# GANtastic3/MaskCycleGAN-VC

Measured on AMD Instinct MI355X. Metric: train iters/s (full G+D step), 80x64 mel bs=1, higher is better.
Workload: dtype f32

## Files before the change

### maskcyclegan-vc_amd/csrc/net.hip

```cpp
#include "mcvc_common.h"
#include "twin.h"
#include "pack.h"
#include "misc.h"
#include "trunk.h"
#include "wino.h"
#include "wino4.h"
#include "sgemm.h"
#include "sampler.h"
#include "audio.h"
#include "vocoder.h"
#include "../../include/mcvc.h"
#include <string.h>
#include <algorithm>
#include <map>
#include <mutex>
#include <vector>

static int g_deterministic = [] { const char* e = getenv("MCVC_DETERMINISTIC"); return (e && atoi(e) != 0) ? 1 : 0; }();
int mcvc_deterministic() { return g_deterministic; }

namespace {

constexpr float kInEps = 1e-5f;

// ... 1020 lines not shown
            PackJob q{}; q.kind = PACK_TRUNK_T; q.param = c.wi[br]; q.dst = c.off_tk; q.Cout = c.Cout; q.Cin = c.Cin; q.KW = c.KW;
            q.ld = c.cout_tot * c.KW; q.co_off = br * c.Cout;
            add_job(t, q, cdiv_i(c.Cin, 32), cdiv_i(c.Cout, 32));
        }
        if (c.igemm && (sets & 4) == 0) {
            PackJob fi{}; fi.kind = PACK_FWD_TAP; fi.param = c.wi[br]; fi.dst = c.off_ifwd; fi.Cout = c.Cout; fi.K = K; fi.ld = c.cout_pk;
            fi.co_off = br * c.Cout; fi.KW = c.KH * c.KW;
            if (fw) add_job(t, fi, cdiv_i(K, 32), cdiv_i(c.Cout, 32));
            t.bytes += 4.0 * fw * 2.0 * c.Cout * K; t.wbytes += 4.0 * fw * c.Cout * K;
        }
        if (c.wino3) {
            PackJob w3{}; w3.kind = PACK_WINO3_D; w3.param = c.wi[br]; w3.dst = c.off_w3; w3.Cout = c.Cout; w3.Cin = c.Cin; w3.ld = c.mg_ld;
            w3.xi_stride = c.w3_xi; w3.co_off = br * c.Cout;
            if (bw) add_job(t, w3, cdiv_i(c.Cin, 256), c.Cout);
            PackJob w3f{}; w3f.kind = PACK_WINO3_F; w3f.param = c.wi[br]; w3f.dst = c.off_w3f; w3f.Cout = c.Cout; w3f.Cin = c.Cin; w3f.ld = c.cout_pk;
            w3f.xi_stride = c.w3f_xi; w3f.co_off = br * c.Cout;
            if (fw) add_job(t, w3f, cdiv_i(c.Cout, 256), c.Cin);
            t.bytes += 4.0 * (fw + bw) * (25.0 + 64.0) * c.Cout * c.Cin; t.wbytes += 4.0 * (fw + bw) * 64.0 * c.Cout * c.Cin;
        }
        if (c.wino3 && w43) {
            PackJob w3{}; w3.kind = PACK_WINO43_D; w3.param = c.wi[br]; w3.dst = c.off_w43; w3.Cout = c.Cout; w3.Cin = c.Cin; w3.ld = c.mg_ld;
            w3.xi_stride = c.w3_xi; w3.co_off = br * c.Cout;
            if (bw) add_job(t, w3, cdiv_i(c.Cin, 256), c.Cout);
            PackJob w3f{}; w3f.kind = PACK_WINO43_F; w3f.param = c.wi[br]; w3f.dst = c.off_w43f; w3f.Cout = c.Cout; w3f.Cin = c.Cin; w3f.ld = c.cout_pk;
            w3f.xi_stride = c.w3f_xi; w3f.co_off = br * c.Cout;
            if (fw) add_job(t, w3f, cdiv_i(c.Cout, 256), c.Cin);
            t.bytes += 4.0 * (fw + bw) * (25.0 + 144.0) * c.Cout * c.Cin; t.wbytes += 4.0 * (fw + bw) * 144.0 * c.Cout * c.Cin;
        }
        if (c.wino && w4) {
            PackJob wf{}; wf.kind = PACK_WINO4_F; wf.param = c.wi[br]; wf.dst = c.off_w4f; wf.Cout = c.Cout; wf.Cin = c.Cin; wf.ld = c.cout_pk;
            wf.xi_stride = c.wf_xi; wf.co_off = br * c.Cout;
            if (fw) add_job(t, wf, cdiv_i(c.Cout, 256), c.Cin);
            PackJob wd{}; wd.kind = PACK_WINO4_D; wd.param = c.wi[br]; wd.dst = c.off_w4d; wd.Cout = c.Cout; wd.Cin = c.Cin; wd.ld = c.cin_pk;
            wd.xi_stride = c.wd_xi; wd.co_off = br * c.Cout;
            if (bw) add_job(t, wd, cdiv_i(c.Cin, 256), c.Cout);
            t.bytes += 4.0 * (fw + bw) * (25.0 + 64.0) * c.Cout * c.Cin; t.wbytes += 4.0 * (fw + bw) * 64.0 * c.Cout * c.Cin;
        }
        if (c.wino && w2) {
            PackJob wf{}; wf.kind = PACK_WINO_F; wf.param = c.wi[br]; wf.dst = c.off_wf; wf.Cout = c.Cout; wf.Cin = c.Cin; wf.ld = c.cout_pk;
            wf.xi_stride = c.wf_xi; wf.co_off = br * c.Cout;
            if (fw) add_job(t, wf, cdiv_i(c.Cout, 256), c.Cin);
            PackJob wd{}; wd.kind = PACK_WINO_D; wd.param = c.wi[br]; wd.dst = c.off_wd; wd.Cout = c.Cout; wd.Cin = c.Cin; wd.ld = c.cin_pk;
            wd.xi_stride = c.wd_xi; wd.co_off = br * c.Cout;
            if (bw) add_job(t, wd, cdiv_i(c.Cin, 256), c.Cout);
            t.bytes += 4.0 * (fw + bw) * (25.0 + 36.0) * c.Cout * c.Cin; t.wbytes += 4.0 * (fw + bw) * 36.0 * c.Cout * c.Cin;
        }
        t.bytes += skip_direct ? 8.0 * c.Cout : 4.0 * ((c.off_tk >= 0 ? 6.0 : 4.0) * c.Cout * K + 2.0 * c.Cout);
        t.wbytes += skip_direct ? 4.0 * c.Cout : 4.0 * ((c.off_tk >= 0 ? 3.0 : 2.0) * c.Cout * K + c.Cout);
    }
}

struct DevPackTable { PackJob* jobs; PackDgradArgs* dga; int njobs, nblocks; double bytes; std::vector<int> used; };

template <class Build>
static const DevPackTable* dev_pack_table(int kind, Build&& build, int* err)
{
    static std::mutex mu;
    static std::map<std::pair<int, int>, DevPackTable> cache;
    int dev = 0;
    if (hipGetDevice(&dev) != hipSuccess) { *err = MCVC_ERR_INVALID; return nullptr; }
    std::lock_guard<std::mutex> lk(mu);
    auto it = cache.find({dev, kind});
    if (it != cache.end()) return &it->second;
    PackTable t;
    build(t);
    DevPackTable d{};
    d.njobs = (int)t.jobs.size(); d.nblocks = t.nblocks; d.bytes = t.bytes;
    hipError_t e = hipMalloc((void**)&d.jobs, t.jobs.size() * sizeof(PackJob));
    if (e == hipSuccess) e = hipMalloc((void**)&d.dga, t.dga.size() * sizeof(PackDgradArgs));
    if (e == hipSuccess) e = hipMemcpy(d.jobs, t.jobs.data(), t.jobs.size() * sizeof(PackJob), hipMemcpyHostToDevice);
    if (e == hipSuccess) e = hipMemcpy(d.dga, t.dga.data(), t.dga.size() * sizeof(PackDgradArgs), hipMemcpyHostToDevice);
    if (e != hipSuccess) { *err = (int)e; return nullptr; }
    for (const PackJob& j : t.jobs) d.used.push_back(j.param);
    return &cache.emplace(std::make_pair(dev, kind), std::move(d)).first->second;
}

static int pack_net(const DevPackTable* t, const float* const* params, float* packed, hipStream_t s)
{
    PackPtrs ptrs{};
    for (int i : t->used) { if (i < 0 || i >= 128) return MCVC_ERR_INVALID; ptrs.p[i] = params[i]; }
    return mcvc_pack_net_launch(t->jobs, t->njobs, t->nblocks, t->dga, ptrs, packed, t->bytes, s);
}

struct DevUpdTable { UpdOwner* owners; PackJob* jobs; PackDgradArgs* dga; int nown, nblocks; double adam_floats, pack_bytes; std::vector<int> used;
                     std::vector<long long> sizes; };

template <class Build, class InRange>
static const DevUpdTable* dev_upd_table(int kind, Build&& build, const long long* numel, int nparams, InRange&& in_range, int* err)
{
    static std::mutex mu;
    static std::map<std::pair<int, int>, DevUpdTable> cache;
    int dev = 0;
    if (hipGetDevice(&dev) != hipSuccess) { *err = MCVC_ERR_INVALID; return nullptr; }
    std::lock_guard<std::mutex> lk(mu);
    auto it = cache.find({dev, kind});
    if (it != cache.end()) return &it->second;
    PackTable t;
    build(t);
    std::vector<PackJob> jobs;
    std::vector<UpdOwner> owners;
    DevUpdTable d{};
    int nblocks = 0;
    for (int prm = 0; prm < nparams && prm < 128; ++prm) {
        std::vector<PackJob> mine;
        for (const PackJob& j : t.jobs) if (j.param == prm) mine.push_back(j);
        if (!in_range(prm)) { if (!mine.empty()) { *err = MCVC_ERR_INVALID; return nullptr; } continue; }
        if (numel[prm] <= 0) { if (!mine.empty()) { *err = MCVC_ERR_INVALID; return nullptr; } continue; }
        UpdOwner o{};
        o.param = prm; o.block0 = nblocks; o.e0 = (int)jobs.size(); o.ne = (int)mine.size();
        bool weight = false;
        for (const PackJob& j : mine) weight = weight || j.kind != PACK_COPY;
        if (!weight) {
            o.flat = 1; o.Cout = (int)numel[prm]; o.Cin = o.taps = 1; o.gx = 1;
            for (const PackJob& j : mine) if (j.Cout != o.Cout) { *err = MCVC_ERR_INVALID; return nullptr; }
            nblocks += cdiv_i(o.Cout, 256);
        } else {
            const PackJob& j0 = mine[0];
            o.Cout = j0.Cout; o.Cin = j0.Cin; o.taps = j0.taps;
            for (const PackJob& j : mine) if (j.kind == PACK_COPY || j.Cout != o.Cout || j.Cin != o.Cin || j.taps != o.taps) { *err = MCVC_ERR_INVALID; return nullptr; }
            for (const PackJob& j : mine) if (j.kind >= PACK_WINO_F && j.kind <= PACK_WINO43_F && j.taps != 25) { *err = MCVC_ERR_INVALID; return nullptr; }
            if ((long long)o.Cout * o.Cin * o.taps != numel[prm]) { *err = MCVC_ERR_INVALID; return nullptr; }
            int cb = 32, ib = 32;
            static const int cb25 = mcvc_knob("MCVC_UPD_CB25", 32);
            if (o.taps == 25) { cb = cb25 == 16 ? 16 : 32; ib = 16; }
            else if (o.taps == 3) ib = 64;
            else if (o.taps == 1) ib = 128;
            else if (o.taps > 25) ib = 16;
            o.CB = cb < o.Cout ? cb : o.Cout; o.IB = ib < o.Cin ? ib : o.Cin;
            if ((size_t)o.CB * mcvc_upd_pitch(o.IB, o.taps) * sizeof(float) > kUpdLds) { *err = MCVC_ERR_INVALID; return nullptr; }
            o.vec4 = ((o.IB * o.taps) % 4 == 0 && (o.Cin % o.IB) == 0 && ((long long)o.Cin * o.taps) % 4 == 0) ? 1 : 0;
            o.gx = cdiv_i(o.Cin, o.IB);
            nblocks += o.gx * cdiv_i(o.Cout, o.CB);
        }
        d.adam_floats += (double)numel[prm];
        for (const PackJob& j : mine) jobs.push_back(j);
        owners.push_back(o);
        d.used.push_back(prm); d.sizes.push_back(numel[prm]);
    }
    if (jobs.size() != t.jobs.size() || owners.empty()) { *err = MCVC_ERR_INVALID; return nullptr; }
    d.nown = (int)owners.size(); d.nblocks = nblocks;
    d.pack_bytes = t.wbytes;
    if (jobs.empty()) jobs.push_back(PackJob{});
    if (t.dga.empty()) t.dga.push_back(PackDgradArgs{});
    hipError_t e = hipMalloc((void**)&d.owners, owners.size() * sizeof(UpdOwner));
    if (e == hipSuccess) e = hipMalloc((void**)&d.jobs, jobs.size() * sizeof(PackJob));
    if (e == hipSuccess) e = hipMalloc((void**)&d.dga, t.dga.size() * sizeof(PackDgradArgs));
    if (e == hipSuccess) e = hipMemcpy(d.owners, owners.data(), owners.size() * sizeof(UpdOwner), hipMemcpyHostToDevice);
    if (e == hipSuccess) e = hipMemcpy(d.jobs, jobs.data(), jobs.size() * sizeof(PackJob), hipMemcpyHostToDevice);
    if (e == hipSuccess) e = hipMemcpy(d.dga, t.dga.data(), t.dga.size() * sizeof(PackDgradArgs), hipMemcpyHostToDevice);
    if (e != hipSuccess) { *err = (int)e; return nullptr; }
    return &cache.emplace(std::make_pair(dev, kind), std::move(d)).first->second;
}

struct UpdOpt { const float* flat; const float* grad; const float* grad2; const float* exp_avg; const float* exp_avg_sq;
                float lr, beta1, beta2, eps; int step; float grad_scale; int zero_grads; };

static int update_net(const DevUpdTable* t, const float* const* params, const long long* numel, float* packed, const UpdOpt& o, hipStream_t s)
{
    for (size_t k = 0; k < t->used.size(); ++k) if (numel[t->used[k]] != t->sizes[k]) return MCVC_ERR_INVALID;
    if (!o.flat || !o.grad || !o.exp_avg || !o.exp_avg_sq || o.step < 1) return MCVC_ERR_INVALID;
    if ((((uintptr_t)o.flat | (uintptr_t)o.grad | (uintptr_t)o.grad2 | (uintptr_t)o.exp_avg | (uintptr_t)o.exp_avg_sq) & 15) != 0) return MCVC_ERR_INVALID;
    PackPtrs ptrs{};
    for (int i : t->used) { if (i < 0 || i >= 128 || !params[i] || (((uintptr_t)params[i]) & 15) != 0) return MCVC_ERR_INVALID; ptrs.p[i] = params[i]; }
    UpdAdam ad{};
    ad.d_g = o.grad - o.flat; ad.d_m = o.exp_avg - o.flat; ad.d_v = o.exp_avg_sq - o.flat;
    ad.has_g2 = o.grad2 ? 1 : 0; ad.d_g2 = o.grad2 ? o.grad2 - o.flat : 0;
    ad.zero = o.zero_grads;
    ad.c = mcvc_adam_coef(o.lr, o.beta1, o.beta2, o.eps, o.step, o.grad_scale);
    const double bytes = (28.0 + (o.grad2 ? 4.0 : 0.0) + (o.zero_grads ? (o.grad2 ? 8.0 : 4.0) : 0.0)) * t->adam_floats + t->pack_bytes;
    return mcvc_update_net_launch(t->owners, t->nown, t->nblocks, t->jobs, t->dga, ptrs, packed, ad, bytes, s);
}

static bool trunk_enabled()
{
    static const int en = mcvc_knob("MCVC_TRUNK", 1);
    return en != 0;
}

static int g_trunk_net = mcvc_knob("MCVC_TRUNK_NET", 1) != 0;
static bool trunk_net_enabled() { return g_trunk_net != 0; }
static bool trunk_bwd_net_enabled() { return g_trunk_net == 1; }

static bool trunk_fwd(Exec& ex, const ConvSpec& c, const float* const* P, int g0, int be0, int g1, int be1, const float* x, float* conv_out,
                      float* stats, float* y, long long y_sn, long long y_sc, const float* res, int B, int W4)
{
    const int mode = (c.nbr == 2) ? TRUNK_IN_GLU : TRUNK_IN;
    if (!trunk_enabled() || c.KH != 1 || !mcvc_trunk_applies(c.Cin, c.KW, c.Cout, B, W4, mode, 1)) return false;
    if (ex.dry) return true;
    TrunkArgs a{};
    a.a0 = P[c.wi[0]]; a.bias0 = P[c.bi[0]]; a.gamma0 = P[g0]; a.beta0 = P[be0];
    if (c.nbr == 2) { a.a1 = P[c.wi[1]]; a.bias1 = P[c.bi[1]]; a.gamma1 = P[g1]; a.beta1 = P[be1]; }
    a.x = x; a.x_sc = (long long)B * W4; a.x_sb = W4;
    a.Cin = c.Cin; a.KW = c.KW; a.K = c.Cin * c.KW; a.M = c.Cout; a.Mtot = c.cout_tot; a.B = B; a.T4 = W4; a.N = B * W4;
    a.conv_out = conv_out; a.c_sc = (long long)B * W4; a.c_sb = W4;
    a.stats = stats; a.y = y; a.res = res; a.y_sn = y_sn; a.y_sc = y_sc; a.eps = kInEps; a.mode = mode;
    ex.fail(mcvc_trunk_launch(a, 1, ex.s));
    return true;
}

static int trunk_pick_ksplit(int Cin, int KW, int M, int B, int W4, int must_split)
{
    int best = 0;
    for (int ks = 1; ks <= 64; ++ks) {
        if (!mcvc_trunk_applies(Cin, KW, M, B, W4, TRUNK_PLAIN, ks)) continue;
        if (best == 0) best = ks;
        if ((M / 16) * ks <= 512) best = ks;
    }
    (void)must_split;
    return best;
}

struct TrunkPre {
    int kind;
    const float* x; const float* stats;
    const float* g0; const float* b0; const float* g1; const float* b1;
    float* out;
    float* dg0; float* db0; float* dg1; float* db1;
    int xB;
};

static bool trunk_dgrad(Exec& ex, const ConvSpec& c, const float* packed, const float* dy, float* dx, int accumulate, int B, int W4,
                        int* nsplit = nullptr, const TrunkPre* pre = nullptr)
{
    if (!trunk_enabled() || c.off_tk < 0) return false;
    int ks = 1;
    if (!accumulate && mcvc_trunk_applies(c.cout_tot, c.KW, c.Cin, B, W4, TRUNK_PLAIN, 1)) ks = 1;
    else ks = trunk_pick_ksplit(c.cout_tot, c.KW, c.Cin, B, W4, 0);
    if (ks < 1) return false;
    if (!accumulate && ks > 1 && !nsplit) return false;
    const long long tot = (long long)c.Cin * B * W4;
    const bool slab_all = accumulate && ks > 1 && nsplit && mcvc_deterministic();
    if (ks > 1 && (!accumulate || nsplit)) {
        const long long need = (long long)(accumulate ? ks : ks - 1) * tot;
        if (need > ex.slab_need) ex.slab_need = need;
        if (!ex.dry && need > ex.slab_cap) { ex.fail(MCVC_ERR_WORKSPACE); return true; }
    }
    if (nsplit) *nsplit = slab_all ? ks + 1 : (accumulate ? 1 : ks);
    if (ex.dry) return true;
    TrunkArgs a{};
    a.a0 = packed + c.off_tk;
    a.x = dy; a.x_sc = (long long)B * W4; a.x_sb = W4;
    a.Cin = c.cout_tot; a.KW = c.KW; a.K = c.cout_tot * c.KW; a.M = c.Cin; a.Mtot = c.Cin; a.B = B; a.T4 = W4; a.N = B * W4;
    a.conv_out = dx; a.c_sc = (long long)B * W4; a.c_sb = W4; a.accumulate = accumulate; a.mode = TRUNK_PLAIN;
    a.slabs = ex.slabs; a.slab_stride = tot; a.slab_all = slab_all ? 1 : 0;
    if (pre) {
        a.pre = pre->kind; a.pre_C = (pre->kind == 2) ? c.cout_tot / 2 : c.cout_tot;
        a.pre_x = pre->x; a.pre_xB = pre->xB; a.pre_stats = pre->stats; a.pre_gamma0 = pre->g0; a.pre_beta0 = pre->b0; a.pre_gamma1 = pre->g1; a.pre_beta1 = pre->b1;
        a.pre_out = pre->out; a.pre_dgamma0 = pre->dg0; a.pre_dbeta0 = pre->db0; a.pre_dgamma1 = pre->dg1; a.pre_dbeta1 = pre->db1;
        wait_readers(ex, pre->out);
    }
    ex.fail(mcvc_trunk_launch(a, ks, ex.s));
    return true;
}
// ... 1612 lines not shown
```

### maskcyclegan-vc_amd/csrc/pack.h

```cpp
#pragma once
#include <hip/hip_runtime.h>

struct DgradClass {
    int nth, ntw;
    int khmax, kwmax;
    int pad_h, pad_w;
    int qh, qw;
    int su, sv;
    long long offset;
};

struct PackDgradArgs {
    int Cin, KH, KW;
    int step;
    int ld;
    int co_off;
    int merged;
    int mg_kh, mg_kw;
    int ncls;
    DgradClass cls[4];
    int tapmajor;
    int cout_rows;
};

int mcvc_pack_fwd_launch(const float* w, float* dst, int Cout, int K, int ld, int co_off, hipStream_t s);
int mcvc_pack_dgrad_launch(const float* w, float* dst, const PackDgradArgs& a, int Cout, hipStream_t s);
int mcvc_copy_launch(const float* src, float* dst, int n, hipStream_t s);

enum PackKind { PACK_FWD = 0, PACK_DGRAD = 1, PACK_COPY = 2, PACK_TRUNK_T = 3, PACK_WINO_F = 4, PACK_WINO_D = 5, PACK_WINO3_D = 6, PACK_WINO3_F = 7, PACK_WINO4_F = 8, PACK_WINO4_D = 9, PACK_WINO43_D = 10, PACK_WINO43_F = 11,
                PACK_FWD_TAP = 12 };
struct PackJob {
    int kind, param;
    int block0, gx;
    long long dst;
    int Cout, K, ld, co_off, KW, Cin;
    int dg;
    int taps;
    long long xi_stride;
};
struct PackPtrs { const float* p[128]; };
constexpr size_t kPackNetLds = 32 * 75 * sizeof(float);
int mcvc_pack_net_launch(const PackJob* d_jobs, int njobs, int nblocks, const PackDgradArgs* d_dga, const PackPtrs& ptrs, float* packed,
                         double bytes, hipStream_t s);
int mcvc_pack_trunk_t_launch(const float* w, float* dst, int Cout, int Cin, int KW, int ld, int co_off, hipStream_t s);

#include "misc.h"
struct UpdOwner {
    int param;
    int block0, gx;
    int Cout, Cin, taps;
    int CB, IB;
    int e0, ne;
    int flat;
    int vec4;
};
struct UpdAdam { long long d_g, d_g2, d_m, d_v; int has_g2, zero; AdamCoef c; };
static inline int mcvc_upd_pitch(int IB, int taps) { return ((IB * taps + 3) & ~3) + 1; }
constexpr size_t kUpdLds = 52 * 1024;
int mcvc_update_net_launch(const UpdOwner* d_owners, int nown, int nblocks, const PackJob* d_jobs, const PackDgradArgs* d_dga, const PackPtrs& ptrs,
                           float* packed, const UpdAdam& ad, double bytes, hipStream_t s);
```

### maskcyclegan-vc_amd/csrc/pack_kernels.hip

```cpp
#include "mcvc_common.h"
#include "pack.h"
#include "trace.h"
#include "launch.h"
#include "wino.h"
#include "wino4.h"

__device__ __forceinline__ void pack_fwd_tile(const float* __restrict__ w, float* __restrict__ dst, int Cout, int K, int ld, int co_off,
                                              int bx, int by, float* smem, int taps = 0)
{
    float (*tile)[33] = reinterpret_cast<float (*)[33]>(smem);
    const int k0 = bx * 32, c0 = by * 32;
    const int tx = threadIdx.x & 31, ty = threadIdx.x >> 5;
    for (int r = ty; r < 32; r += 8) {
        const int co = c0 + r, k = k0 + tx;
        tile[r][tx] = (co < Cout && k < K) ? w[(long long)co * K + k] : 0.f;
    }
    __syncthreads();
    for (int r = ty; r < 32; r += 8) {
        const int k = k0 + r, co = c0 + tx;
        if (k < K && co < Cout) {
            const int row = taps > 0 ? (k % taps) * (K / taps) + k / taps : k;
            dst[(long long)row * ld + co_off + co] = tile[tx][r];
        }
    }
}

__device__ __forceinline__ void pack_dgrad_tile(const float* __restrict__ w, float* __restrict__ dst, const PackDgradArgs& a, int bx, int by,
                                                float* lds)
{
    const int ci0 = bx * 32, co = by;
    const int khkw = a.KH * a.KW;
    int nci = a.Cin - ci0; if (nci > 32) nci = 32;
    const float* src = w + ((long long)co * a.Cin + ci0) * khkw;
    for (int i = threadIdx.x; i < nci * khkw; i += 256) lds[i] = src[i];
    __syncthreads();
    const int lane = threadIdx.x & 31, grp = threadIdx.x >> 5;
    for (int c = 0; c < a.ncls; ++c) {
        const int nt = a.cls[c].nth * a.cls[c].ntw;
        for (int t = grp; t < nt; t += 8) {
            const int u = t / a.cls[c].ntw, v = t - u * a.cls[c].ntw;
            const int kh = a.cls[c].khmax - a.step * u, kw = a.cls[c].kwmax - a.step * v;
            if (lane < nci) {
                const float wv = lds[lane * khkw + kh * a.KW + kw];
                if (a.tapmajor) {
                    dst[a.cls[c].offset + ((long long)t * a.cout_rows + a.co_off + co) * a.ld + ci0 + lane] = wv;
                } else if (a.merged) {
                    const long long row = ((long long)(a.co_off + co) * a.mg_kh + (u + a.cls[c].su)) * a.mg_kw + (v + a.cls[c].sv);
                    dst[row * a.ld + 4 * (ci0 + lane) + 2 * a.cls[c].qh + a.cls[c].qw] = wv;
                } else {
                    dst[a.cls[c].offset + ((long long)(a.co_off + co) * nt + t) * a.ld + ci0 + lane] = wv;
                }
            }
        }
    }
}

__device__ __forceinline__ void pack_trunk_t_tile(const float* __restrict__ w, float* __restrict__ dst, int Cout, int Cin, int KW, int ld,
                                                  int co_off, int bx, int by, float* smem)
{
    float (*tile)[33] = reinterpret_cast<float (*)[33]>(smem);
    const int ci0 = bx * 32, co0 = by * 32;
    const int tx = threadIdx.x & 31, ty = threadIdx.x >> 5;
    for (int kw = 0; kw < KW; ++kw) {
        for (int r = ty; r < 32; r += 8) {
            const int co = co0 + r, ci = ci0 + tx;
            tile[r][tx] = (co < Cout && ci < Cin) ? w[((long long)co * Cin + ci) * KW + kw] : 0.f;
        }
        __syncthreads();
        for (int r = ty; r < 32; r += 8) {
            const int ci = ci0 + r, co = co0 + tx;
            if (ci < Cin && co < Cout) dst[(long long)ci * ld + (long long)(co_off + co) * KW + (KW - 1 - kw)] = tile[tx][r];
        }
        __syncthreads();
    }
}

__global__ void __launch_bounds__(256) pack_fwd_kernel(const float* __restrict__ w, float* __restrict__ dst, int Cout, int K, int ld, int co_off)
{
    __shared__ float smem[32 * 33];
    pack_fwd_tile(w, dst, Cout, K, ld, co_off, blockIdx.x, blockIdx.y, smem);
}

__global__ void __launch_bounds__(256) pack_dgrad_kernel(const float* __restrict__ w, float* __restrict__ dst, PackDgradArgs a)
{
    extern __shared__ float lds[];
    pack_dgrad_tile(w, dst, a, blockIdx.x, blockIdx.y, lds);
}

__global__ void __launch_bounds__(256) pack_trunk_t_kernel(const float* __restrict__ w, float* __restrict__ dst, int Cout, int Cin, int KW, int ld,
                                                           int co_off)
{
    __shared__ float smem[32 * 33];
    pack_trunk_t_tile(w, dst, Cout, Cin, KW, ld, co_off, blockIdx.x, blockIdx.y, smem);
}

struct CopyKArgs { const float* src; float* dst; int n; };
__global__ void copy_kernel(const Twin<CopyKArgs> tw)
{
    const CopyKArgs ka_ = tw.v[blockIdx.z];
    const float* __restrict__ src = ka_.src;
    float* __restrict__ dst = ka_.dst;
    int n = ka_.n;
    const int i = blockIdx.x * blockDim.x + threadIdx.x;
    if (i < n) dst[i] = src[i];
}

struct PackNetKArgs { const PackJob* jobs; int njobs; const PackDgradArgs* dga; PackPtrs ptrs; float* packed; };
__global__ void __launch_bounds__(256) pack_net_kernel(const Twin<PackNetKArgs> tw)
{
    const PackNetKArgs& ka_ = tw.v[blockIdx.z];
    const PackJob* __restrict__ jobs = ka_.jobs;
    int njobs = ka_.njobs;
    const PackDgradArgs* __restrict__ dga = ka_.dga;
    const PackPtrs& ptrs = ka_.ptrs;
    float* __restrict__ packed = ka_.packed;
    extern __shared__ float lds[];
    const int blk = blockIdx.x;
    int lo = 0, hi = njobs - 1;
    while (lo < hi) { const int mid = (lo + hi + 1) >> 1; if (jobs[mid].block0 <= blk) lo = mid; else hi = mid - 1; }
    const PackJob j = jobs[lo];
    const int rel = blk - j.block0;
    const int bx = rel % j.gx, by = rel / j.gx;
    const float* w = ptrs.p[j.param];
    float* dst = packed + j.dst;
    switch (j.kind) {
    case PACK_FWD: pack_fwd_tile(w, dst, j.Cout, j.K, j.ld, j.co_off, bx, by, lds); break;
    case PACK_FWD_TAP: pack_fwd_tile(w, dst, j.Cout, j.K, j.ld, j.co_off, bx, by, lds, j.KW); break;
    case PACK_DGRAD: pack_dgrad_tile(w, dst, dga[j.dg], bx, by, lds); break;
    case PACK_TRUNK_T: pack_trunk_t_tile(w, dst, j.Cout, j.Cin, j.KW, j.ld, j.co_off, bx, by, lds); break;
    case PACK_WINO_F: wino_weight_tile(w, dst, j.Cout, j.Cin, j.ld, j.xi_stride, j.co_off, 0, bx, by); break;
    case PACK_WINO_D: wino_weight_tile(w, dst, j.Cout, j.Cin, j.ld, j.xi_stride, j.co_off, 1, bx, by); break;
    case PACK_WINO3_D: wino3_weight_tile(w, dst, j.Cout, j.Cin, j.ld, j.xi_stride, j.co_off, bx, by); break;
    case PACK_WINO3_F: wino3_weight_fwd_tile(w, dst, j.Cout, j.Cin, j.ld, j.xi_stride, j.co_off, bx, by); break;
    case PACK_WINO4_F: wino4_weight_tile(w, dst, j.Cout, j.Cin, j.ld, j.xi_stride, j.co_off, 0, bx, by); break;
    case PACK_WINO4_D: wino4_weight_tile(w, dst, j.Cout, j.Cin, j.ld, j.xi_stride, j.co_off, 1, bx, by); break;
    case PACK_WINO43_D: wino3_weight_tile_p<6>(w, dst, j.Cout, j.Cin, j.ld, j.xi_stride, j.co_off, bx, by); break;
    case PACK_WINO43_F: wino3_weight_fwd_tile_p<6>(w, dst, j.Cout, j.Cin, j.ld, j.xi_stride, j.co_off, bx, by); break;
    default: { const int i = rel * 256 + threadIdx.x; if (i < j.Cout) dst[i] = w[i]; } break;
    }
}

struct UpdTile { const float* lds; int pitch, taps, co0, ci0, nc, ni, CB, IB, Cin; };

__device__ __forceinline__ void upd_emit_fwd(const PackJob& j, float* __restrict__ dst, const UpdTile& t, bool tapmajor)
{
    const int nk = t.ni * t.taps;
    for (int idx = threadIdx.x; idx < nk * t.CB; idx += 256) {
        const int c = idx % t.CB, kl = idx / t.CB;
        if (c >= t.nc) continue;
        const int i = kl / t.taps, tp = kl - i * t.taps;
        const int ci = t.ci0 + i;
        const long long row = tapmajor ? (long long)tp * t.Cin + ci : (long long)ci * t.taps + tp;
        dst[row * j.ld + j.co_off + t.co0 + c] = t.lds[c * t.pitch + kl];
    }
}

__device__ __forceinline__ void upd_emit_dgrad(float* __restrict__ dst, const PackDgradArgs& a, const UpdTile& t)
{
    for (int cl = 0; cl < a.ncls; ++cl) {
        const DgradClass& k = a.cls[cl];
        const int nt = k.nth * k.ntw;
        const int total = nt * t.nc * t.IB;
        for (int idx = threadIdx.x; idx < total; idx += 256) {
            const int i = idx % t.IB, r = idx / t.IB;
            if (i >= t.ni) continue;
            const int c = r % t.nc, tp = r / t.nc;
            const int u = tp / k.ntw, v = tp - u * k.ntw;
            const int kh = k.khmax - a.step * u, kw = k.kwmax - a.step * v;
            const float wv = t.lds[c * t.pitch + i * t.taps + kh * a.KW + kw];
            const int co = t.co0 + c, ci = t.ci0 + i;
            if (a.tapmajor) {
                dst[k.offset + ((long long)tp * a.cout_rows + a.co_off + co) * a.ld + ci] = wv;
            } else if (a.merged) {
                const long long row = ((long long)(a.co_off + co) * a.mg_kh + (u + k.su)) * a.mg_kw + (v + k.sv);
                dst[row * a.ld + 4 * ci + 2 * k.qh + k.qw] = wv;
            } else {
                dst[k.offset + ((long long)(a.co_off + co) * nt + tp) * a.ld + ci] = wv;
            }
        }
    }
}

__device__ __forceinline__ void upd_emit_trunk_t(const PackJob& j, float* __restrict__ dst, const UpdTile& t)
{
    const int KW = t.taps, span = t.nc * KW;
    for (int idx = threadIdx.x; idx < span * t.ni; idx += 256) {
        const int q = idx % span, i = idx / span;
        const int c = q / KW, kwp = q - c * KW;
        dst[(long long)(t.ci0 + i) * j.ld + (long long)(j.co_off + t.co0) * KW + q] = t.lds[c * t.pitch + i * KW + (KW - 1 - kwp)];
    }
}

template <class F>
__device__ __forceinline__ void upd_emit_filters(const UpdTile& t, bool along_co, F&& f)
{
    const int nf = t.nc * t.ni;
    for (int q = threadIdx.x; q < nf; q += 256) {
        const int c = along_co ? q % t.nc : q / t.ni, i = along_co ? q / t.nc : q % t.ni;
        f(t.lds + c * t.pitch + i * 25, t.co0 + c, t.ci0 + i);
    }
}

struct UpdNetKArgs { const UpdOwner* owners; int nown; const PackJob* jobs; const PackDgradArgs* dga; PackPtrs ptrs; float* packed; UpdAdam ad; };
__global__ void __launch_bounds__(256) update_net_kernel(const Twin<UpdNetKArgs> tw)
{
    const UpdNetKArgs& ka_ = tw.v[blockIdx.z];
    const UpdOwner* __restrict__ owners = ka_.owners;
    const PackJob* __restrict__ jobs = ka_.jobs;
    const PackDgradArgs* __restrict__ dga = ka_.dga;
    float* __restrict__ packed = ka_.packed;
    const UpdAdam ad = ka_.ad;
    extern __shared__ __attribute__((aligned(16))) float lds[];
    const int blk = blockIdx.x;
    int lo = 0, hi = ka_.nown - 1;
    while (lo < hi) { const int mid = (lo + hi + 1) >> 1; if (owners[mid].block0 <= blk) lo = mid; else hi = mid - 1; }
    const UpdOwner o = owners[lo];
    const int rel = blk - o.block0;
    float* __restrict__ p = const_cast<float*>(ka_.ptrs.p[o.param]);
    float* __restrict__ g = p + ad.d_g;
    float* __restrict__ g2 = ad.has_g2 ? p + ad.d_g2 : nullptr;
    float* __restrict__ m = p + ad.d_m;
    float* __restrict__ v = p + ad.d_v;
    const AdamCoef c = ad.c;
    if (o.flat) {
        const int i = rel * 256 + threadIdx.x;
        if (i >= o.Cout) return;
        float gr = g[i];
        if (g2) gr += g2[i];
        if (ad.zero) { g[i] = 0.f; if (g2) g2[i] = 0.f; }
        float pn = p[i], mn = m[i], vn = v[i];
        adam_elem(pn, gr, mn, vn, c);
        p[i] = pn; m[i] = mn; v[i] = vn;
        for (int e = 0; e < o.ne; ++e) packed[jobs[o.e0 + e].dst + i] = pn;
        return;
    }
    const int bx = rel % o.gx, by = rel / o.gx;
    UpdTile t;
    t.lds = lds; t.taps = o.taps; t.CB = o.CB; t.IB = o.IB; t.Cin = o.Cin;
    t.co0 = by * o.CB; t.ci0 = bx * o.IB;
    t.nc = min(o.CB, o.Cout - t.co0); t.ni = min(o.IB, o.Cin - t.ci0);
    const int run = t.ni * o.taps;
    t.pitch = ((o.IB * o.taps + 3) & ~3) + 1;
    const long long row_stride = (long long)o.Cin * o.taps;
    const long long base = (long long)t.co0 * row_stride + (long long)t.ci0 * o.taps;
    if (o.vec4) {
        const int run4 = run >> 2, total4 = t.nc * run4;
        constexpr int U = 2;
        for (int q0 = threadIdx.x; q0 < total4; q0 += U * 256) {
            float4 pp[U], gg[U], hh[U], mm[U], vv[U];
            long long off[U]; int ldo[U]; bool ok[U];
#pragma unroll
            for (int u = 0; u < U; ++u) {
                const int q = q0 + u * 256;
                ok[u] = q < total4;
                const int qq = ok[u] ? q : 0;
                const int cc = qq / run4, r4 = qq - cc * run4;
                off[u] = base + cc * row_stride + 4 * r4;
                ldo[u] = cc * t.pitch + 4 * r4;
                pp[u] = *reinterpret_cast<const float4*>(p + off[u]);
                gg[u] = *reinterpret_cast<const float4*>(g + off[u]);
                hh[u] = g2 ? *reinterpret_cast<const float4*>(g2 + off[u]) : make_float4(0.f, 0.f, 0.f, 0.f);
                mm[u] = *reinterpret_cast<const float4*>(m + off[u]);
                vv[u] = *reinterpret_cast<const float4*>(v + off[u]);
            }
#pragma unroll
            for (int u = 0; u < U; ++u) {
                if (!ok[u]) continue;
                if (g2) { gg[u].x += hh[u].x; gg[u].y += hh[u].y; gg[u].z += hh[u].z; gg[u].w += hh[u].w; }
                if (ad.zero) {
                    *reinterpret_cast<float4*>(g + off[u]) = make_float4(0.f, 0.f, 0.f, 0.f);
                    if (g2) *reinterpret_cast<float4*>(g2 + off[u]) = make_float4(0.f, 0.f, 0.f, 0.f);
                }
                float* pf = reinterpret_cast<float*>(&pp[u]);
                float* gf = reinterpret_cast<float*>(&gg[u]);
                float* mf = reinterpret_cast<float*>(&mm[u]);
                float* vf = reinterpret_cast<float*>(&vv[u]);
#pragma unroll
                for (int k = 0; k < 4; ++k) adam_elem(pf[k], gf[k], mf[k], vf[k], c);
                *reinterpret_cast<float4*>(p + off[u]) = pp[u];
                *reinterpret_cast<float4*>(m + off[u]) = mm[u];
                *reinterpret_cast<float4*>(v + off[u]) = vv[u];
                lds[ldo[u]] = pp[u].x; lds[ldo[u] + 1] = pp[u].y; lds[ldo[u] + 2] = pp[u].z; lds[ldo[u] + 3] = pp[u].w;
            }
        }
    } else {
        const int total = t.nc * run;
        for (int q = threadIdx.x; q < total; q += 256) {
            const int cc = q / run, r = q - cc * run;
            const long long off = base + cc * row_stride + r;
            float gr = g[off];
            if (g2) gr += g2[off];
            if (ad.zero) { g[off] = 0.f; if (g2) g2[off] = 0.f; }
            float pn = p[off], mn = m[off], vn = v[off];
            adam_elem(pn, gr, mn, vn, c);
            p[off] = pn; m[off] = mn; v[off] = vn;
            lds[cc * t.pitch + r] = pn;
        }
    }
    if (o.ne == 0) return;
    __syncthreads();
    for (int e = 0; e < o.ne; ++e) {
        const PackJob j = jobs[o.e0 + e];
        float* dst = packed + j.dst;
        switch (j.kind) {
        case PACK_FWD: upd_emit_fwd(j, dst, t, false); break;
        case PACK_FWD_TAP: upd_emit_fwd(j, dst, t, true); break;
        case PACK_DGRAD: upd_emit_dgrad(dst, dga[j.dg], t); break;
        case PACK_TRUNK_T: upd_emit_trunk_t(j, dst, t); break;
        case PACK_WINO_F: upd_emit_filters(t, true, [&](const float* f, int co, int ci) { wino_weight_core(f, dst, co, ci, j.ld, j.xi_stride, j.co_off, 0); }); break;
        case PACK_WINO_D: upd_emit_filters(t, false, [&](const float* f, int co, int ci) { wino_weight_core(f, dst, co, ci, j.ld, j.xi_stride, j.co_off, 1); }); break;
        case PACK_WINO3_D: upd_emit_filters(t, false, [&](const float* f, int co, int ci) { wino3_weight_core_p<4>(f, dst, co, ci, j.ld, j.xi_stride, j.co_off); }); break;
        case PACK_WINO3_F: upd_emit_filters(t, true, [&](const float* f, int co, int ci) { wino3_weight_fwd_core_p<4>(f, dst, co, ci, j.ld, j.xi_stride, j.co_off); }); break;
        case PACK_WINO4_F: upd_emit_filters(t, true, [&](const float* f, int co, int ci) { wino4_weight_core(f, dst, co, ci, j.ld, j.xi_stride, j.co_off, 0); }); break;
        case PACK_WINO4_D: upd_emit_filters(t, false, [&](const float* f, int co, int ci) { wino4_weight_core(f, dst, co, ci, j.ld, j.xi_stride, j.co_off, 1); }); break;
        case PACK_WINO43_D: upd_emit_filters(t, false, [&](const float* f, int co, int ci) { wino3_weight_core_p<6>(f, dst, co, ci, j.ld, j.xi_stride, j.co_off); }); break;
        case PACK_WINO43_F: upd_emit_filters(t, true, [&](const float* f, int co, int ci) { wino3_weight_fwd_core_p<6>(f, dst, co, ci, j.ld, j.xi_stride, j.co_off); }); break;
        default: break;
        }
    }
}

int mcvc_update_net_launch(const UpdOwner* d_owners, int nown, int nblocks, const PackJob* d_jobs, const PackDgradArgs* d_dga, const PackPtrs& ptrs,
                           float* packed, const UpdAdam& ad, double bytes, hipStream_t s)
{
    TraceScope ts(K_ADAM, s, 0.0, bytes);
    mcvc_launch(update_net_kernel, dim3((unsigned)nblocks), dim3(256), kUpdLds, s, UpdNetKArgs{d_owners, nown, d_jobs, d_dga, ptrs, packed, ad});
    return (int)hipGetLastError();
}

int mcvc_pack_net_launch(const PackJob* d_jobs, int njobs, int nblocks, const PackDgradArgs* d_dga, const PackPtrs& ptrs, float* packed,
                         double bytes, hipStream_t s)
{
    TraceScope ts(K_PACK, s, 0.0, bytes);
    mcvc_launch(pack_net_kernel, dim3((unsigned)nblocks), dim3(256), kPackNetLds, s, PackNetKArgs{d_jobs, njobs, d_dga, ptrs, packed});
    return (int)hipGetLastError();
}

int mcvc_pack_trunk_t_launch(const float* w, float* dst, int Cout, int Cin, int KW, int ld, int co_off, hipStream_t s)
{
    dim3 grid((unsigned)cdiv_i(Cin, 32), (unsigned)cdiv_i(Cout, 32));
    TraceScope ts(K_PACK, s, 0.0, 8.0 * (double)Cout * Cin * KW);
    hipLaunchKernelGGL(pack_trunk_t_kernel, grid, dim3(256), 0, s, w, dst, Cout, Cin, KW, ld, co_off);
    return (int)hipGetLastError();
}

int mcvc_pack_fwd_launch(const float* w, float* dst, int Cout, int K, int ld, int co_off, hipStream_t s)
{
    dim3 grid((unsigned)cdiv_i(K, 32), (unsigned)cdiv_i(Cout, 32));
    TraceScope ts(K_PACK, s, 0.0, 8.0 * (double)Cout * K);
    hipLaunchKernelGGL(pack_fwd_kernel, grid, dim3(256), 0, s, w, dst, Cout, K, ld, co_off);
    return (int)hipGetLastError();
}

int mcvc_pack_dgrad_launch(const float* w, float* dst, const PackDgradArgs& a, int Cout, hipStream_t s)
{
    dim3 grid((unsigned)cdiv_i(a.Cin, 32), (unsigned)Cout);
    const size_t lds = (size_t)32 * a.KH * a.KW * sizeof(float);
    TraceScope ts(K_PACK, s, 0.0, 8.0 * (double)Cout * a.Cin * a.KH * a.KW);
    hipLaunchKernelGGL(pack_dgrad_kernel, grid, dim3(256), lds, s, w, dst, a);
    return (int)hipGetLastError();
}

int mcvc_copy_launch(const float* src, float* dst, int n, hipStream_t s)
{
    TraceScope ts(K_ELEMENTWISE, s, 0.0, 8.0 * n);
    mcvc_launch(copy_kernel, dim3((unsigned)cdiv_i(n, 256)), dim3(256), 0, s, CopyKArgs{src, dst, n});
    return (int)hipGetLastError();
}
```

Before: 178.6.

## Restructure fused Adam+repack kernel: block map, LDS descriptors, vectorised tails, smaller LDS

Reworks the fused optimizer-update-and-repack kernel. A per-block owner map replaces the binary search, and flat params are handled four elements per thread with a scalar tail. Job and dgrad descriptors are staged into LDS and read uniformly with readfirstlane. Vectorised loads now also cover contiguous tiles, and the dynamic LDS allocation is sized to the largest tile actually used. Tile sizes shrink for small 25-tap and large-tap layers to raise the block count. The intent is to cut scalar memory traffic and index overhead and to improve occupancy in the per-step update, at the cost of more complex descriptor handling and new validation limits.

```diff
diff --git a/maskcyclegan-vc_amd/csrc/net.hip b/maskcyclegan-vc_amd/csrc/net.hip
--- a/maskcyclegan-vc_amd/csrc/net.hip
+++ b/maskcyclegan-vc_amd/csrc/net.hip
@@ -1126,8 +1126,8 @@
     return mcvc_pack_net_launch(t->jobs, t->njobs, t->nblocks, t->dga, ptrs, packed, t->bytes, s);
 }
 
-struct DevUpdTable { UpdOwner* owners; PackJob* jobs; PackDgradArgs* dga; int nown, nblocks; double adam_floats, pack_bytes; std::vector<int> used;
-                     std::vector<long long> sizes; };
+struct DevUpdTable { UpdOwner* owners; int* map; PackJob* jobs; PackDgradArgs* dga; int nown, nblocks; size_t lds; double adam_floats, pack_bytes;
+                     std::vector<int> used; std::vector<long long> sizes; };
 
 template <class Build, class InRange>
 static const DevUpdTable* dev_upd_table(int kind, Build&& build, const long long* numel, int nparams, InRange&& in_range, int* err)
@@ -1142,9 +1142,12 @@
     PackTable t;
     build(t);
     std::vector<PackJob> jobs;
+    std::vector<PackDgradArgs> dga;
     std::vector<UpdOwner> owners;
+    std::vector<int> map;
     DevUpdTable d{};
     int nblocks = 0;
+    size_t tile_bytes = 0;
     for (int prm = 0; prm < nparams && prm < 128; ++prm) {
         std::vector<PackJob> mine;
         for (const PackJob& j : t.jobs) if (j.param == prm) mine.push_back(j);
@@ -1152,46 +1155,74 @@
         if (numel[prm] <= 0) { if (!mine.empty()) { *err = MCVC_ERR_INVALID; return nullptr; } continue; }
         UpdOwner o{};
         o.param = prm; o.block0 = nblocks; o.e0 = (int)jobs.size(); o.ne = (int)mine.size();
+        o.fdst = -1;
         bool weight = false;
         for (const PackJob& j : mine) weight = weight || j.kind != PACK_COPY;
+        int nb = 0;
         if (!weight) {
             o.flat = 1; o.Cout = (int)numel[prm]; o.Cin = o.taps = 1; o.gx = 1;
-            for (const PackJob& j : mine) if (j.Cout != o.Cout) { *err = MCVC_ERR_INVALID; return nullptr; }
-            nblocks += cdiv_i(o.Cout, 256);
+            if (mine.size() > 1) { *err = MCVC_ERR_INVALID; return nullptr; }
+            for (const PackJob& j : mine) { if (j.Cout != o.Cout) { *err = MCVC_ERR_INVALID; return nullptr; } o.fdst = j.dst; }
+            nb = cdiv_i(o.Cout, kUpdFlat);
         } else {
             const PackJob& j0 = mine[0];
             o.Cout = j0.Cout; o.Cin = j0.Cin; o.taps = j0.taps;
             for (const PackJob& j : mine) if (j.kind == PACK_COPY || j.Cout != o.Cout || j.Cin != o.Cin || j.taps != o.taps) { *err = MCVC_ERR_INVALID; return nullptr; }
             for (const PackJob& j : mine) if (j.kind >= PACK_WINO_F && j.kind <= PACK_WINO43_F && j.taps != 25) { *err = MCVC_ERR_INVALID; return nullptr; }
             if ((long long)o.Cout * o.Cin * o.taps != numel[prm]) { *err = MCVC_ERR_INVALID; return nullptr; }
+            if (o.ne > kUpdMaxEmits) { *err = MCVC_ERR_INVALID; return nullptr; }
             int cb = 32, ib = 32;
             static const int cb25 = mcvc_knob("MCVC_UPD_CB25", 32);
-            if (o.taps == 25) { cb = cb25 == 16 ? 16 : 32; ib = 16; }
+            if (o.taps == 25) {
+                cb = cb25 == 16 ? 16 : 32; ib = 16;
+                if (cdiv_i(o.Cout, 32) * cdiv_i(o.Cin, 16) < 256) cb = 16;
+            }
             else if (o.taps == 3) ib = 64;
             else if (o.taps == 1) ib = 128;
-            else if (o.taps > 25) ib = 16;
+            else if (o.taps > 25) { ib = 16; cb = 4; }
             o.CB = cb < o.Cout ? cb : o.Cout; o.IB = ib < o.Cin ? ib : o.Cin;
-            if ((size_t)o.CB * mcvc_upd_pitch(o.IB, o.taps) * sizeof(float) > kUpdLds) { *err = MCVC_ERR_INVALID; return nullptr; }
-            o.vec4 = ((o.IB * o.taps) % 4 == 0 && (o.Cin % o.IB) == 0 && ((long long)o.Cin * o.taps) % 4 == 0) ? 1 : 0;
+            const size_t tb = (size_t)o.CB * mcvc_upd_pitch(o.IB, o.taps) * sizeof(float);
+            if (tb + kUpdHdrWords * sizeof(float) > kUpdLds) { *err = MCVC_ERR_INVALID; return nullptr; }
+            if (tb > tile_bytes) tile_bytes = tb;
+            const long long run = (long long)o.IB * o.taps;
+            const bool rows4 = run % 4 == 0 && (o.Cin % o.IB) == 0 && ((long long)o.Cin * o.taps) % 4 == 0;
+            const bool contig4 = o.IB == o.Cin && run >= 4 && ((long long)o.CB * run) % 4 == 0;
+            o.vec4 = (rows4 || contig4) ? 1 : 0;
             o.gx = cdiv_i(o.Cin, o.IB);
-            nblocks += o.gx * cdiv_i(o.Cout, o.CB);
+            nb = o.gx * cdiv_i(o.Cout, o.CB);
         }
         d.adam_floats += (double)numel[prm];
-        for (const PackJob& j : mine) jobs.push_back(j);
+        o.dg0 = (int)dga.size();
+        for (PackJob j : mine) {
+            if (j.kind == PACK_DGRAD) {
+                if (j.dg < 0 || j.dg >= (int)t.dga.size()) { *err = MCVC_ERR_INVALID; return nullptr; }
+                dga.push_back(t.dga[j.dg]);
+                j.dg = (int)dga.size() - 1;
+                ++o.ndg;
+            }
+            jobs.push_back(j);
+        }
+        if (o.ndg == 0) o.dg0 = 0;
+        if (o.ndg > kUpdMaxDg) { *err = MCVC_ERR_INVALID; return nullptr; }
+        map.insert(map.end(), (size_t)nb, (int)owners.size());
+        nblocks += nb;
         owners.push_back(o);
         d.used.push_back(prm); d.sizes.push_back(numel[prm]);
     }
-    if (jobs.size() != t.jobs.size() || owners.empty()) { *err = MCVC_ERR_INVALID; return nullptr; }
+    if (jobs.size() != t.jobs.size() || owners.empty() || (int)map.size() != nblocks) { *err = MCVC_ERR_INVALID; return nullptr; }
     d.nown = (int)owners.size(); d.nblocks = nblocks;
+    d.lds = kUpdHdrWords * sizeof(float) + tile_bytes;
     d.pack_bytes = t.wbytes;
     if (jobs.empty()) jobs.push_back(PackJob{});
-    if (t.dga.empty()) t.dga.push_back(PackDgradArgs{});
+    if (dga.empty()) dga.push_back(PackDgradArgs{});
     hipError_t e = hipMalloc((void**)&d.owners, owners.size() * sizeof(UpdOwner));
+    if (e == hipSuccess) e = hipMalloc((void**)&d.map, map.size() * sizeof(int));
     if (e == hipSuccess) e = hipMalloc((void**)&d.jobs, jobs.size() * sizeof(PackJob));
-    if (e == hipSuccess) e = hipMalloc((void**)&d.dga, t.dga.size() * sizeof(PackDgradArgs));
+    if (e == hipSuccess) e = hipMalloc((void**)&d.dga, dga.size() * sizeof(PackDgradArgs));
     if (e == hipSuccess) e = hipMemcpy(d.owners, owners.data(), owners.size() * sizeof(UpdOwner), hipMemcpyHostToDevice);
+    if (e == hipSuccess) e = hipMemcpy(d.map, map.data(), map.size() * sizeof(int), hipMemcpyHostToDevice);
     if (e == hipSuccess) e = hipMemcpy(d.jobs, jobs.data(), jobs.size() * sizeof(PackJob), hipMemcpyHostToDevice);
-    if (e == hipSuccess) e = hipMemcpy(d.dga, t.dga.data(), t.dga.size() * sizeof(PackDgradArgs), hipMemcpyHostToDevice);
+    if (e == hipSuccess) e = hipMemcpy(d.dga, dga.data(), dga.size() * sizeof(PackDgradArgs), hipMemcpyHostToDevice);
     if (e != hipSuccess) { *err = (int)e; return nullptr; }
     return &cache.emplace(std::make_pair(dev, kind), std::move(d)).first->second;
 }
@@ -1212,7 +1243,7 @@
     ad.zero = o.zero_grads;
     ad.c = mcvc_adam_coef(o.lr, o.beta1, o.beta2, o.eps, o.step, o.grad_scale);
     const double bytes = (28.0 + (o.grad2 ? 4.0 : 0.0) + (o.zero_grads ? (o.grad2 ? 8.0 : 4.0) : 0.0)) * t->adam_floats + t->pack_bytes;
-    return mcvc_update_net_launch(t->owners, t->nown, t->nblocks, t->jobs, t->dga, ptrs, packed, ad, bytes, s);
+    return mcvc_update_net_launch(t->owners, t->map, t->nblocks, t->lds, t->jobs, t->dga, ptrs, packed, ad, bytes, s);
 }
 
 static bool trunk_enabled()
diff --git a/maskcyclegan-vc_amd/csrc/pack.h b/maskcyclegan-vc_amd/csrc/pack.h
--- a/maskcyclegan-vc_amd/csrc/pack.h
+++ b/maskcyclegan-vc_amd/csrc/pack.h
@@ -51,11 +51,19 @@
     int Cout, Cin, taps;
     int CB, IB;
     int e0, ne;
+    int dg0, ndg;
     int flat;
     int vec4;
+    long long fdst;
 };
 struct UpdAdam { long long d_g, d_g2, d_m, d_v; int has_g2, zero; AdamCoef c; };
 static inline int mcvc_upd_pitch(int IB, int taps) { return ((IB * taps + 3) & ~3) + 1; }
-constexpr size_t kUpdLds = 52 * 1024;
-int mcvc_update_net_launch(const UpdOwner* d_owners, int nown, int nblocks, const PackJob* d_jobs, const PackDgradArgs* d_dga, const PackPtrs& ptrs,
-                           float* packed, const UpdAdam& ad, double bytes, hipStream_t s);
+constexpr int kUpdFlat = 1024;
+constexpr int kUpdMaxEmits = 12, kUpdMaxDg = 2;
+constexpr int kUpdJobWords = sizeof(PackJob) / 4, kUpdDgWords = sizeof(PackDgradArgs) / 4;
+static_assert(sizeof(PackJob) % 4 == 0 && sizeof(PackDgradArgs) % 4 == 0 && kUpdMaxEmits * kUpdJobWords <= 256 && kUpdMaxDg * kUpdDgWords <= 256,
+              "one descriptor word per thread of a 256-thread workgroup");
+constexpr int kUpdHdrWords = (kUpdMaxEmits * kUpdJobWords + kUpdMaxDg * kUpdDgWords + 3) & ~3;
+constexpr size_t kUpdLds = 52 * 1024 + kUpdHdrWords * sizeof(float);
+int mcvc_update_net_launch(const UpdOwner* d_owners, const int* d_map, int nblocks, size_t lds, const PackJob* d_jobs, const PackDgradArgs* d_dga,
+                           const PackPtrs& ptrs, float* packed, const UpdAdam& ad, double bytes, hipStream_t s);
diff --git a/maskcyclegan-vc_amd/csrc/pack_kernels.hip b/maskcyclegan-vc_amd/csrc/pack_kernels.hip
--- a/maskcyclegan-vc_amd/csrc/pack_kernels.hip
+++ b/maskcyclegan-vc_amd/csrc/pack_kernels.hip
@@ -4,6 +4,7 @@
 #include "launch.h"
 #include "wino.h"
 #include "wino4.h"
+#include <cstddef>
 
 __device__ __forceinline__ void pack_fwd_tile(const float* __restrict__ w, float* __restrict__ dst, int Cout, int K, int ld, int co_off,
                                               int bx, int by, float* smem, int taps = 0)
@@ -155,10 +156,27 @@
     }
 }
 
-__device__ __forceinline__ void upd_emit_dgrad(float* __restrict__ dst, const PackDgradArgs& a, const UpdTile& t)
-{
+template <class D>
+__device__ __forceinline__ D upd_desc(const int* words)
+{
+    struct W { int w[sizeof(D) / 4]; } t;
+#pragma unroll
+    for (int k = 0; k < (int)(sizeof(D) / 4); ++k) t.w[k] = __builtin_amdgcn_readfirstlane(words[k]);
+    D d;
+    __builtin_memcpy(&d, &t, sizeof(D));
+    return d;
+}
+
+struct PackDgradHead { int Cin, KH, KW, step, ld, co_off, merged, mg_kh, mg_kw, ncls; };
+static_assert(offsetof(PackDgradArgs, cls) == sizeof(PackDgradHead) && offsetof(PackDgradArgs, ncls) == offsetof(PackDgradHead, ncls) &&
+              sizeof(DgradClass) % 4 == 0 && offsetof(PackDgradArgs, cout_rows) == offsetof(PackDgradArgs, tapmajor) + 4, "PackDgradArgs layout");
+__device__ __forceinline__ void upd_emit_dgrad(float* __restrict__ dst, const int* aw, const UpdTile& t)
+{
+    const PackDgradHead a = upd_desc<PackDgradHead>(aw);
+    struct Tail { int tapmajor, cout_rows; };
+    const Tail z = upd_desc<Tail>(aw + offsetof(PackDgradArgs, tapmajor) / 4);
     for (int cl = 0; cl < a.ncls; ++cl) {
-        const DgradClass& k = a.cls[cl];
+        const DgradClass k = upd_desc<DgradClass>(aw + (offsetof(PackDgradArgs, cls) + cl * sizeof(DgradClass)) / 4);
         const int nt = k.nth * k.ntw;
         const int total = nt * t.nc * t.IB;
         for (int idx = threadIdx.x; idx < total; idx += 256) {
@@ -169,8 +187,8 @@
             const int kh = k.khmax - a.step * u, kw = k.kwmax - a.step * v;
             const float wv = t.lds[c * t.pitch + i * t.taps + kh * a.KW + kw];
             const int co = t.co0 + c, ci = t.ci0 + i;
-            if (a.tapmajor) {
-                dst[k.offset + ((long long)tp * a.cout_rows + a.co_off + co) * a.ld + ci] = wv;
+            if (z.tapmajor) {
+                dst[k.offset + ((long long)tp * z.cout_rows + a.co_off + co) * a.ld + ci] = wv;
             } else if (a.merged) {
                 const long long row = ((long long)(a.co_off + co) * a.mg_kh + (u + k.su)) * a.mg_kw + (v + k.sv);
                 dst[row * a.ld + 4 * ci + 2 * k.qh + k.qw] = wv;
@@ -201,7 +219,47 @@
     }
 }
 
-struct UpdNetKArgs { const UpdOwner* owners; int nown; const PackJob* jobs; const PackDgradArgs* dga; PackPtrs ptrs; float* packed; UpdAdam ad; };
+struct UpdBufs { float* __restrict__ p; float* __restrict__ g; float* __restrict__ g2; float* __restrict__ m; float* __restrict__ v; };
+struct UpdQuad { float4 p, g, h, m, v; };
+__device__ __forceinline__ UpdQuad upd_load4(const UpdBufs& b, long long off)
+{
+    UpdQuad q;
+    q.p = *reinterpret_cast<const float4*>(b.p + off);
+    q.g = *reinterpret_cast<const float4*>(b.g + off);
+    q.h = b.g2 ? *reinterpret_cast<const float4*>(b.g2 + off) : make_float4(0.f, 0.f, 0.f, 0.f);
+    q.m = *reinterpret_cast<const float4*>(b.m + off);
+    q.v = *reinterpret_cast<const float4*>(b.v + off);
+    return q;
+}
+__device__ __forceinline__ void upd_step4(const UpdBufs& b, long long off, UpdQuad& q, const UpdAdam& ad)
+{
+    if (b.g2) { q.g.x += q.h.x; q.g.y += q.h.y; q.g.z += q.h.z; q.g.w += q.h.w; }
+    if (ad.zero) {
+        *reinterpret_cast<float4*>(b.g + off) = make_float4(0.f, 0.f, 0.f, 0.f);
+        if (b.g2) *reinterpret_cast<float4*>(b.g2 + off) = make_float4(0.f, 0.f, 0.f, 0.f);
+    }
+    float* pf = reinterpret_cast<float*>(&q.p);
+    float* gf = reinterpret_cast<float*>(&q.g);
+    float* mf = reinterpret_cast<float*>(&q.m);
+    float* vf = reinterpret_cast<float*>(&q.v);
+#pragma unroll
+    for (int k = 0; k < 4; ++k) adam_elem(pf[k], gf[k], mf[k], vf[k], ad.c);
+    *reinterpret_cast<float4*>(b.p + off) = q.p;
+    *reinterpret_cast<float4*>(b.m + off) = q.m;
+    *reinterpret_cast<float4*>(b.v + off) = q.v;
+}
+__device__ __forceinline__ float upd_step1(const UpdBufs& b, long long off, const UpdAdam& ad)
+{
+    float gr = b.g[off];
+    if (b.g2) gr += b.g2[off];
+    if (ad.zero) { b.g[off] = 0.f; if (b.g2) b.g2[off] = 0.f; }
+    float pn = b.p[off], mn = b.m[off], vn = b.v[off];
+    adam_elem(pn, gr, mn, vn, ad.c);
+    b.p[off] = pn; b.m[off] = mn; b.v[off] = vn;
+    return pn;
+}
+
+struct UpdNetKArgs { const UpdOwner* owners; const int* map; const PackJob* jobs; const PackDgradArgs* dga; PackPtrs ptrs; float* packed; UpdAdam ad; };
 __global__ void __launch_bounds__(256) update_net_kernel(const Twin<UpdNetKArgs> tw)
 {
     const UpdNetKArgs& ka_ = tw.v[blockIdx.z];
@@ -210,30 +268,38 @@
     const PackDgradArgs* __restrict__ dga = ka_.dga;
     float* __restrict__ packed = ka_.packed;
     const UpdAdam ad = ka_.ad;
-    extern __shared__ __attribute__((aligned(16))) float lds[];
-    const int blk = blockIdx.x;
-    int lo = 0, hi = ka_.nown - 1;
-    while (lo < hi) { const int mid = (lo + hi + 1) >> 1; if (owners[mid].block0 <= blk) lo = mid; else hi = mid - 1; }
-    const UpdOwner o = owners[lo];
-    const int rel = blk - o.block0;
-    float* __restrict__ p = const_cast<float*>(ka_.ptrs.p[o.param]);
-    float* __restrict__ g = p + ad.d_g;
-    float* __restrict__ g2 = ad.has_g2 ? p + ad.d_g2 : nullptr;
-    float* __restrict__ m = p + ad.d_m;
-    float* __restrict__ v = p + ad.d_v;
-    const AdamCoef c = ad.c;
+    extern __shared__ __attribute__((aligned(16))) float lds_all[];
+    const int tid = threadIdx.x;
+    const UpdOwner o = owners[ka_.map[blockIdx.x]];
+    const int rel = blockIdx.x - o.block0;
+    UpdBufs b;
+    b.p = const_cast<float*>(ka_.ptrs.p[o.param]);
+    b.g = b.p + ad.d_g;
+    b.g2 = ad.has_g2 ? b.p + ad.d_g2 : nullptr;
+    b.m = b.p + ad.d_m;
+    b.v = b.p + ad.d_v;
     if (o.flat) {
-        const int i = rel * 256 + threadIdx.x;
-        if (i >= o.Cout) return;
-        float gr = g[i];
-        if (g2) gr += g2[i];
-        if (ad.zero) { g[i] = 0.f; if (g2) g2[i] = 0.f; }
-        float pn = p[i], mn = m[i], vn = v[i];
-        adam_elem(pn, gr, mn, vn, c);
-        p[i] = pn; m[i] = mn; v[i] = vn;
-        for (int e = 0; e < o.ne; ++e) packed[jobs[o.e0 + e].dst + i] = pn;
+        const int n = o.Cout, n4 = n >> 2;
+        float* __restrict__ cp = o.fdst >= 0 ? packed + o.fdst : nullptr;
+        const int i4 = rel * 256 + tid;
+        if (i4 < n4) {
+            const int i = 4 * i4;
+            UpdQuad q = upd_load4(b, i);
+            upd_step4(b, i, q, ad);
+            if (cp) { cp[i] = q.p.x; cp[i + 1] = q.p.y; cp[i + 2] = q.p.z; cp[i + 3] = q.p.w; }
+        }
+        const int it = 4 * n4 + tid;
+        if (rel == (n - 1) / kUpdFlat && it < n) {
+            const float pn = upd_step1(b, it, ad);
+            if (cp) cp[it] = pn;
+        }
         return;
     }
+    int* hdr = reinterpret_cast<int*>(lds_all);
+    float* lds = lds_all + kUpdHdrWords;
+    const int njw = o.ne * kUpdJobWords, ndw = o.ndg * kUpdDgWords;
+    const int jw = reinterpret_cast<const int*>(jobs + o.e0)[min(tid, max(njw, 1) - 1)];
+    const int dw = reinterpret_cast<const int*>(dga + o.dg0)[min(tid, max(ndw, 1) - 1)];
     const int bx = rel % o.gx, by = rel / o.gx;
     UpdTile t;
     t.lds = lds; t.taps = o.taps; t.CB = o.CB; t.IB = o.IB; t.Cin = o.Cin;
@@ -243,69 +309,52 @@
     t.pitch = ((o.IB * o.taps + 3) & ~3) + 1;
     const long long row_stride = (long long)o.Cin * o.taps;
     const long long base = (long long)t.co0 * row_stride + (long long)t.ci0 * o.taps;
+    const int total = t.nc * run;
+    int done = 0;
     if (o.vec4) {
-        const int run4 = run >> 2, total4 = t.nc * run4;
+        const int total4 = total >> 2;
+        done = 4 * total4;
         constexpr int U = 2;
-        for (int q0 = threadIdx.x; q0 < total4; q0 += U * 256) {
-            float4 pp[U], gg[U], hh[U], mm[U], vv[U];
-            long long off[U]; int ldo[U]; bool ok[U];
+        for (int q0 = tid; q0 < total4; q0 += U * 256) {
+            UpdQuad qd[U];
+            long long off[U]; int ldo[U], room[U]; bool ok[U];
 #pragma unroll
             for (int u = 0; u < U; ++u) {
                 const int q = q0 + u * 256;
                 ok[u] = q < total4;
-                const int qq = ok[u] ? q : 0;
-                const int cc = qq / run4, r4 = qq - cc * run4;
-                off[u] = base + cc * row_stride + 4 * r4;
-                ldo[u] = cc * t.pitch + 4 * r4;
-                pp[u] = *reinterpret_cast<const float4*>(p + off[u]);
-                gg[u] = *reinterpret_cast<const float4*>(g + off[u]);
-                hh[u] = g2 ? *reinterpret_cast<const float4*>(g2 + off[u]) : make_float4(0.f, 0.f, 0.f, 0.f);
-                mm[u] = *reinterpret_cast<const float4*>(m + off[u]);
-                vv[u] = *reinterpret_cast<const float4*>(v + off[u]);
+                const int f = ok[u] ? 4 * q : 0;
+                const int cc = f / run, r = f - cc * run;
+                off[u] = base + cc * row_stride + r;
+                ldo[u] = cc * t.pitch + r;
+                room[u] = run - r;
+                qd[u] = upd_load4(b, off[u]);
             }
 #pragma unroll
             for (int u = 0; u < U; ++u) {
                 if (!ok[u]) continue;
-                if (g2) { gg[u].x += hh[u].x; gg[u].y += hh[u].y; gg[u].z += hh[u].z; gg[u].w += hh[u].w; }
-                if (ad.zero) {
-                    *reinterpret_cast<float4*>(g + off[u]) = make_float4(0.f, 0.f, 0.f, 0.f);
-                    if (g2) *reinterpret_cast<float4*>(g2 + off[u]) = make_float4(0.f, 0.f, 0.f, 0.f);
-                }
-                float* pf = reinterpret_cast<float*>(&pp[u]);
-                float* gf = reinterpret_cast<float*>(&gg[u]);
-                float* mf = reinterpret_cast<float*>(&mm[u]);
-                float* vf = reinterpret_cast<float*>(&vv[u]);
-#pragma unroll
-                for (int k = 0; k < 4; ++k) adam_elem(pf[k], gf[k], mf[k], vf[k], c);
-                *reinterpret_cast<float4*>(p + off[u]) = pp[u];
-                *reinterpret_cast<float4*>(m + off[u]) = mm[u];
-                *reinterpret_cast<float4*>(v + off[u]) = vv[u];
-                lds[ldo[u]] = pp[u].x; lds[ldo[u] + 1] = pp[u].y; lds[ldo[u] + 2] = pp[u].z; lds[ldo[u] + 3] = pp[u].w;
+                upd_step4(b, off[u], qd[u], ad);
+                const int skip = t.pitch - run;
+                lds[ldo[u]] = qd[u].p.x;
+                lds[ldo[u] + 1 + (room[u] > 1 ? 0 : skip)] = qd[u].p.y;
+                lds[ldo[u] + 2 + (room[u] > 2 ? 0 : skip)] = qd[u].p.z;
+                lds[ldo[u] + 3 + (room[u] > 3 ? 0 : skip)] = qd[u].p.w;
             }
         }
-    } else {
-        const int total = t.nc * run;
-        for (int q = threadIdx.x; q < total; q += 256) {
-            const int cc = q / run, r = q - cc * run;
-            const long long off = base + cc * row_stride + r;
-            float gr = g[off];
-            if (g2) gr += g2[off];
-            if (ad.zero) { g[off] = 0.f; if (g2) g2[off] = 0.f; }
-            float pn = p[off], mn = m[off], vn = v[off];
-            adam_elem(pn, gr, mn, vn, c);
-            p[off] = pn; m[off] = mn; v[off] = vn;
-            lds[cc * t.pitch + r] = pn;
-        }
-    }
-    if (o.ne == 0) return;
+    }
+    for (int q = done + tid; q < total; q += 256) {
+        const int cc = q / run, r = q - cc * run;
+        lds[cc * t.pitch + r] = upd_step1(b, base + cc * row_stride + r, ad);
+    }
+    if (tid < njw) hdr[tid] = jw;
+    if (tid < ndw) hdr[kUpdMaxEmits * kUpdJobWords + tid] = dw;
     __syncthreads();
     for (int e = 0; e < o.ne; ++e) {
-        const PackJob j = jobs[o.e0 + e];
+        const PackJob j = upd_desc<PackJob>(hdr + e * kUpdJobWords);
         float* dst = packed + j.dst;
         switch (j.kind) {
         case PACK_FWD: upd_emit_fwd(j, dst, t, false); break;
         case PACK_FWD_TAP: upd_emit_fwd(j, dst, t, true); break;
-        case PACK_DGRAD: upd_emit_dgrad(dst, dga[j.dg], t); break;
+        case PACK_DGRAD: upd_emit_dgrad(dst, hdr + kUpdMaxEmits * kUpdJobWords + (j.dg - o.dg0) * kUpdDgWords, t); break;
         case PACK_TRUNK_T: upd_emit_trunk_t(j, dst, t); break;
         case PACK_WINO_F: upd_emit_filters(t, true, [&](const float* f, int co, int ci) { wino_weight_core(f, dst, co, ci, j.ld, j.xi_stride, j.co_off, 0); }); break;
         case PACK_WINO_D: upd_emit_filters(t, false, [&](const float* f, int co, int ci) { wino_weight_core(f, dst, co, ci, j.ld, j.xi_stride, j.co_off, 1); }); break;
@@ -320,11 +369,11 @@
     }
 }
 
-int mcvc_update_net_launch(const UpdOwner* d_owners, int nown, int nblocks, const PackJob* d_jobs, const PackDgradArgs* d_dga, const PackPtrs& ptrs,
-                           float* packed, const UpdAdam& ad, double bytes, hipStream_t s)
+int mcvc_update_net_launch(const UpdOwner* d_owners, const int* d_map, int nblocks, size_t lds, const PackJob* d_jobs, const PackDgradArgs* d_dga,
+                           const PackPtrs& ptrs, float* packed, const UpdAdam& ad, double bytes, hipStream_t s)
 {
     TraceScope ts(K_ADAM, s, 0.0, bytes);
-    mcvc_launch(update_net_kernel, dim3((unsigned)nblocks), dim3(256), kUpdLds, s, UpdNetKArgs{d_owners, nown, d_jobs, d_dga, ptrs, packed, ad});
+    mcvc_launch(update_net_kernel, dim3((unsigned)nblocks), dim3(256), lds, s, UpdNetKArgs{d_owners, d_map, d_jobs, d_dga, ptrs, packed, ad});
     return (int)hipGetLastError();
 }
 
```

Result: no change. 178.7 (median of 2 runs) (+0.1%).
